# RishWijewardhena/vision-textile-inspection

Hardware: AMD Instinct MI355X
Metric: frames/sec whole-node, YOLOv8n-seg 640x640 bs=64; mask IoU vs CPU ref (higher is better)
Workload: dtype f16x2

## Files before the change

vision-textile-inspection_amd/csrc/conv_dev.h:

```cpp
#pragma once
#include "vti_internal.h"

namespace vti {

typedef _Float16 half_t;
typedef _Float16 half8 __attribute__((ext_vector_type(8)));
typedef _Float16 half4 __attribute__((ext_vector_type(4)));
typedef float f32x4 __attribute__((ext_vector_type(4)));

typedef unsigned u32x4 __attribute__((ext_vector_type(4)));

struct h2_t { unsigned u; };
struct h2x4 { u32x4 u; };
constexpr float H2_SX = 16.0f;

template <typename T> struct Tr;
template <> struct Tr<half_t> { typedef half8 vec; static constexpr int VEC = 8, KC = 32; static constexpr bool H16 = true, F32 = false, H2 = false; };
template <> struct Tr<float> { typedef f32x4 vec; static constexpr int VEC = 4, KC = 16; static constexpr bool H16 = false, F32 = true, H2 = false; };
template <> struct Tr<h2_t> { typedef h2x4 vec; static constexpr int VEC = 4, KC = 16; static constexpr bool H16 = false, F32 = false, H2 = true; };

typedef _Float16 half2v __attribute__((ext_vector_type(2)));
__device__ __forceinline__ unsigned h2_enc(float v) {
    half2v p;
    p[0] = (half_t)__builtin_fmaf(v, H2_SX, 0.0f);
// ... 20 lines not shown
    if constexpr (Tr<T>::H2) return (f32x4){h2_dec(u[0]), h2_dec(u[1]), h2_dec(u[2]), h2_dec(u[3])};
    else return __builtin_bit_cast(f32x4, u);
}
template <typename T> __device__ __forceinline__ f32x4 acc_bias(f32x4 acc, f32x4 bias, float alpha) {
    if constexpr (Tr<T>::H2) return acc * (f32x4){alpha, alpha, alpha, alpha} + bias;
    else return acc + bias;
}

__device__ __forceinline__ f32x4 mma(half8 w, half8 x, f32x4 c) {
    return __builtin_amdgcn_mfma_f32_16x16x32_f16(w, x, c, 0, 0, 0);
}
__device__ __forceinline__ f32x4 mma(f32x4 w, f32x4 x, f32x4 c) {
    c = __builtin_amdgcn_mfma_f32_16x16x4f32(w[0], x[0], c, 0, 0, 0);
    c = __builtin_amdgcn_mfma_f32_16x16x4f32(w[1], x[1], c, 0, 0, 0);
    c = __builtin_amdgcn_mfma_f32_16x16x4f32(w[2], x[2], c, 0, 0, 0);
    c = __builtin_amdgcn_mfma_f32_16x16x4f32(w[3], x[3], c, 0, 0, 0);
    return c;
}

__device__ __forceinline__ f32x4 mma(h2x4 w, h2x4 x, f32x4 c) {
    u32x4 wh, wl;
#pragma unroll
    for (int i = 0; i < 4; ++i) {
        wh[i] = __builtin_amdgcn_perm(w.u[i], w.u[i], 0x01000100u);
        wl[i] = w.u[i] >> 16;
    }
    const half8 xv = __builtin_bit_cast(half8, x.u);
    c = __builtin_amdgcn_mfma_f32_16x16x32_f16(__builtin_bit_cast(half8, wh), xv, c, 0, 0, 0);
    c = __builtin_amdgcn_mfma_f32_16x16x32_f16(__builtin_bit_cast(half8, wl), xv, c, 0, 0, 0);
    return c;
}

template <int NREP, int M, int TAPS, int XD, class LDX, class LDW>
__device__ __forceinline__ void h2_taps(f32x4 (&acc)[M][NREP], LDX ldx, LDW ldw) {
    constexpr int NSTEP = TAPS * M;
    constexpr unsigned SEL_H = 0x01000100u;
    h2x4 xq[XD];
    u32x4 wraw[NREP];
    u32x4 wh[2][NREP], wl[2][NREP];
#pragma unroll
    for (int n = 0; n < NREP; ++n) wraw[n] = ldw(0, n).u;
#pragma unroll
    for (int i = 0; i < XD - 1; ++i) xq[i] = ldx(i);
#pragma unroll
    for (int n = 0; n < NREP; ++n)
#pragma unroll
        for (int i = 0; i < 4; ++i) {
            wh[0][n][i] = __builtin_amdgcn_perm(wraw[n][i], wraw[n][i], SEL_H);
            wl[0][n][i] = wraw[n][i] >> 16;
        }
#pragma unroll
    for (int s_ = 0; s_ < NSTEP; ++s_) {
        const int tp = s_ / M, mm = s_ % M, cur = tp & 1, nxt = cur ^ 1;
#ifdef H2_EXP_NOXREAD
        if (s_ + XD - 1 < NSTEP && s_ < XD) xq[(s_ + XD - 1) % XD] = ldx(s_ + XD - 1);
#else
        if (s_ + XD - 1 < NSTEP) xq[(s_ + XD - 1) % XD] = ldx(s_ + XD - 1);
#endif
        if (mm == 0 && tp + 1 < TAPS) {
#pragma unroll
            for (int n = 0; n < NREP; ++n) wraw[n] = ldw(tp + 1, n).u;
        }
        __builtin_amdgcn_sched_barrier(0);
        const half8 xv = __builtin_bit_cast(half8, xq[s_ % XD].u);
#pragma unroll
        for (int j = 0; j < 2 * NREP; ++j) {
            const int n = j >> 1;
// ... 510 lines not shown
```

vision-textile-inspection_amd/csrc/conv_pk.hip:

```cpp
#include <algorithm>
#include <cstdlib>
#include <type_traits>

#include "conv_dev.h"

namespace vti {

constexpr int PK_PWP = 24;
constexpr int PK_TW = 20;
constexpr int PK_ROWS = 4;
constexpr int PK_MAXD = 9;
constexpr int PK_MAXD2 = 13;

using ConvPkS1 = Combos<Ints<1, 1>, Ints<2, 1>, Ints<3, 1>, Ints<4, 1>, Ints<5, 1>, Ints<1, 2>, Ints<2, 2>, Ints<3, 2>, Ints<4, 2>, Ints<1, 4>,
                        Ints<2, 4>>;
using ConvPkS2 = Combos<Ints<1, 4>, Ints<2, 2>, Ints<4, 1>, Ints<2, 1>, Ints<1, 2>>;
using Conv1Pk = decltype(concat(ConvPkS1{}, Combos<Ints<4, 4>>{}));
bool conv_pk_instantiated(int nrep, int wn) { return combo_has(ConvPkS1{}, nrep, wn); }
bool conv_pk2_instantiated(int nrep, int wn) { return combo_has(ConvPkS2{}, nrep, wn); }
bool conv1_pk_instantiated(int nrep, int wn) { return combo_has(Conv1Pk{}, nrep, wn); }
using Conv1PkWH2 = Combos<Ints<2, 2, 4>, Ints<2, 2, 6>, Ints<2, 2, 8>, Ints<2, 2, 12>, Ints<2, 2, 16>,
                          Ints<2, 4, 4>, Ints<2, 4, 6>, Ints<2, 4, 8>, Ints<2, 4, 12>, Ints<2, 4, 16>>;
using Conv1PkWF16 = Combos<Ints<2, 2, 2>, Ints<2, 2, 3>, Ints<2, 2, 4>, Ints<2, 2, 6>, Ints<2, 2, 8>,
                           Ints<2, 4, 2>, Ints<2, 4, 3>, Ints<2, 4, 4>, Ints<2, 4, 6>, Ints<2, 4, 8>, Ints<4, 1, 2>>;
// ... 20 lines not shown
static int pk_ring_depth(int maxd, int per_step, F lds_at) {
    int d = 2;
    while (d < maxd && lds_at(d + 1) <= 160 * 1024 && per_step * (d - 1) <= 63) ++d;
    return d;
}
static int pk3_depth(int S, int TH, int WN, int NREP, int nchunks, int wstat, int maxd) {
    if (!pk3_fits(S, TH, WN, NREP, nchunks, wstat)) return 0;
    const int ncomp = (TH / PK_ROWS) * WN;
    const int per_step = ((int)(pk_stage_bytes(TH, S) / 1024) + ncomp - 1) / ncomp + (nchunks > 2 && !wstat ? (WN * NREP * 9 + ncomp - 1) / ncomp : 0);
    return pk_ring_depth(maxd, per_step, [&](int d) { return pk3_lds_bytes(S, TH, WN, NREP, nchunks, d, wstat); });
}
size_t conv_pk_lds_bytes(int TH, int WN, int NREP, int nchunks, int depth, int wstat) { return pk3_lds_bytes(1, TH, WN, NREP, nchunks, depth, wstat); }
size_t conv_pk2_lds_bytes(int TH, int WN, int NREP, int nchunks, int depth, int wstat) { return pk3_lds_bytes(2, TH, WN, NREP, nchunks, depth, wstat); }
bool conv_pk_fits(int TH, int WN, int NREP, int nchunks, int wstat) { return pk3_fits(1, TH, WN, NREP, nchunks, wstat); }
bool conv_pk2_fits(int TH, int WN, int NREP, int nchunks, int wstat) { return pk3_fits(2, TH, WN, NREP, nchunks, wstat); }
int conv_pk_depth(int TH, int WN, int NREP, int nchunks, int wstat, int maxd) { return pk3_depth(1, TH, WN, NREP, nchunks, wstat, maxd); }
int conv_pk2_depth(int TH, int WN, int NREP, int nchunks, int wstat, int maxd) { return pk3_depth(2, TH, WN, NREP, nchunks, wstat, maxd); }

__device__ __forceinline__ void dma16(__amdgpu_buffer_rsrc_t r, unsigned voff, unsigned soff, unsigned lds_addr) {
    unsigned keep;
    asm volatile("s_mov_b32 %0, m0\n\ts_mov_b32 m0, %1\n\ts_nop 0\n\tbuffer_load_dwordx4 %2, %3, %4 offen lds\n\ts_mov_b32 m0, %0"
                 : "=&s"(keep) : "s"(lds_addr), "v"(voff), "s"(r), "s"(soff) : "memory");
}

template <int N> __device__ __forceinline__ void wait_vm() { asm volatile("s_waitcnt vmcnt(%0)" :: "i"(N) : "memory"); }
template <int N> struct WaitVm { static __device__ __forceinline__ void go(int n) { if (n >= N) wait_vm<N>(); else WaitVm<N - 1>::go(n); } };
template <> struct WaitVm<0> { static __device__ __forceinline__ void go(int) { wait_vm<0>(); } };

__device__ __forceinline__ void pk_stagger_wait(int units) {
    if (units > 0 && (int)(blockIdx.x >> 3) * 2 >= (int)(gridDim.x >> 3))
        for (int i = 0; i < units; ++i) __builtin_amdgcn_s_sleep(16);
}

template <typename T, int NREP, int WN, int NREP2 = 0, bool FOLD = false, int S = 1>
__global__ __launch_bounds__(512) void conv3_pk(const ConvParams p) {
    using vec = typename Tr<T>::vec;
    constexpr int VEC = Tr<T>::VEC, KC = Tr<T>::KC, ES = (int)sizeof(T);
    constexpr int TAPS = FOLD ? 4 : 9, NTB = WN * NREP;
    constexpr int PWP = S == 2 ? 2 * PK_PWP : PK_PWP;
    constexpr int MAXD = S == 2 ? PK_MAXD2 : PK_MAXD;
    static_assert(S == 1 || (S == 2 && !FOLD && NREP2 == 0), "stride 2: plain epilogue only");
    constexpr int WCHUNK = NTB * TAPS * 1024;
    constexpr unsigned OOB = 0x80000000u;
    constexpr bool FAST = !Tr<T>::F32;
    extern __shared__ __attribute__((aligned(16))) char smem[];

    const int tid = threadIdx.x, lane = tid & 63;
    const int wave = __builtin_amdgcn_readfirstlane(tid >> 6);
    static_assert(!FOLD || (WN == 4 && NREP2 > 0), "fold: one compute wave per output phase, fused 1x1 epilogue");
    const int ncomp = (p.TH / PK_ROWS) * WN;
    const int nld = (int)(blockDim.x >> 6) - ncomp;
    const int PH = S == 2 ? 2 * p.TH + 1 : p.TH + 2;
    const int stage_bytes = PH * PWP * 64;
    const int ndma = PH * PWP / 16;
    const int D = p.pk_depth;
    const bool stream_w = p.nchunks > 2 && !p.pk_wstat;
    const int wbuf_off = D * stage_bytes;
    const int bias_off = wbuf_off + (stream_w ? D : p.nchunks) * WCHUNK;
    const unsigned lds0 = (unsigned)(size_t)(__attribute__((address_space(3))) char*)smem;
    const int nt0 = blockIdx.y * NTB;

    for (int i = tid; i < NTB * 16; i += (int)blockDim.x) ((float*)(smem + bias_off))[i] = p.bias[nt0 * 16 + i];
    __syncthreads();

    int t, tend, tstride;
    if (p.pk_xcd) {
        const int per = (p.pk_tiles + 7) >> 3, k = blockIdx.x & 7;
        t = k * per + (int)(blockIdx.x >> 3);
        tend = min((k + 1) * per, p.pk_tiles);
        tstride = (int)(gridDim.x >> 3);
    } else {
        t = blockIdx.x; tend = p.pk_tiles; tstride = (int)gridDim.x;
    }
    if (t >= tend) return;
    auto tile_coords = [&](int tt, int& b, int& oy0, int& ox0) {
        const int tx = tt % p.tiles_x, r = tt / p.tiles_x;
        const int ty = r % p.tiles_y;
        b = r / p.tiles_y; oy0 = ty * p.TH; ox0 = tx * PK_TW;
    };
    const int nsteps = ((tend - t + tstride - 1) / tstride) * p.nchunks;

    if (wave >= ncomp) {
        const int lw = wave - ncomp;
        const int q = (lane & 3) ^ (((lane >> 4) & 1) << 1);
        const int cvalid = (p.Cin - q * VEC + KC - 1) / KC;
        int dyx[MAXD];
#pragma unroll
        for (int u = 0; u < MAXD; ++u) {
            const int s = (lw + u * nld) * 16 + (lane >> 2);
            if constexpr (S == 2) {
                const int py = (int)(((unsigned)s * 1366u) >> 16), r = s - py * PWP;
                const int plane = r >= PK_PWP ? 1 : 0, idx = r - plane * PK_PWP;
                dyx[u] = idx < PK_TW + 1 - plane ? (py << 8) | (2 * idx + plane) : -1;
            } else {
                const int py = (int)(((unsigned)s * 2731u) >> 16), px = s - py * PK_PWP;
                dyx[u] = px < PK_TW + 2 ? (py << 8) | px : -1;
            }
        }
        const __amdgpu_buffer_rsrc_t rsA = __builtin_amdgcn_make_buffer_rsrc((void*)p.in, 0, (int)p.in_bytes, 0x00020000);
        const __amdgpu_buffer_rsrc_t rsB = __builtin_amdgcn_make_buffer_rsrc((void*)p.wpk, 0, (int)p.wpk_bytes, 0x00020000);
        unsigned voff[MAXD];
        auto setup_voff = [&](int tt) {
            int b, oy0, ox0;
            tile_coords(tt, b, oy0, ox0);
#pragma unroll
            for (int u = 0; u < MAXD; ++u) {
                const int y = S * oy0 - 1 + (dyx[u] >> 8), x = S * ox0 - 1 + (dyx[u] & 255);
                const bool ok = dyx[u] >= 0 && (unsigned)y < (unsigned)p.Hin && (unsigned)x < (unsigned)p.Win;
                voff[u] = ok ? (unsigned)((((b * p.Hin + y) * p.Win + x) * p.in_ld + p.in_coff + q * VEC) * ES) : OOB;
            }
        };
        auto issue_patch = [&](int c, int stage) {
            const bool qok = c < cvalid;
            const unsigned dst = lds0 + stage * stage_bytes + lw * 1024;
#pragma unroll
            for (int u = 0; u < MAXD; ++u)
// ... 9 lines not shown
        int per_step = 0;
#pragma unroll
        for (int u = 0; u < MAXD; ++u) per_step += (lw + u * nld < ndma) ? 1 : 0;
        if (stream_w && lw < NTB * TAPS) per_step += (NTB * TAPS - lw + nld - 1) / nld;
        int it = t, ic = 0;
        setup_voff(t);
        auto issue_next = [&](int s) {
            const int stage = s % D;
            issue_patch(ic, stage);
            if (stream_w) issue_weights(ic, stage);
            if (++ic == p.nchunks) {
                ic = 0; it += tstride;
                if (it < tend) setup_voff(it);
            }
        };
        const int ahead = min(D - 1, nsteps);
        for (int s = 0; s < ahead; ++s) issue_next(s);
        int w1cnt = 0;
        if (!stream_w) {
            for (int c = 1; c < p.nchunks; ++c) {
                issue_weights(c, c);
                if (lw < NTB * TAPS) w1cnt += (NTB * TAPS - lw + nld - 1) / nld;
            }
        }
        for (int s = 0; s < nsteps; ++s) {
            const int inflight = min(D - 2, nsteps - 1 - s);
            WaitVm<63>::go(min(63, inflight * per_step + (s == 0 ? w1cnt : 0)));
            __builtin_amdgcn_s_barrier();
            if (s + D - 1 < nsteps) issue_next(s + D - 1);
        }
        return;
    }

    const int wn = wave % WN, wm = wave / WN;
    const int fpy = FOLD ? (wn >> 1) : 0, fpx = FOLD ? (wn & 1) : 0;
    int xa[MREP][3], ry[MREP], rx[MREP];
#pragma unroll
    for (int m = 0; m < MREP; ++m) {
        const int pp = m * 16 + (lane & 15), li = lane & 15;
        const int py = p.pk_lin ? (pp * 205) >> 12 : (m < 4 ? m : li >> 2);
        const int px = p.pk_lin ? pp - py * PK_TW : (m < 4 ? li : 16 + (li & 3));
        ry[m] = wm * PK_ROWS + py; rx[m] = px;
#pragma unroll
        for (int dx = 0; dx < 3; ++dx) {
            const int s = S == 2 ? (2 * ry[m]) * PWP + (dx == 1 ? PK_PWP + px : px + (dx >> 1))
                                 : (ry[m] + fpy) * PK_PWP + px + fpx + dx;
            xa[m][dx] = (s * 64 + (lane >> 4) * 16) ^ ((s & 4) << 3);
        }
    }
    const __amdgpu_buffer_rsrc_t rsO = __builtin_amdgcn_make_buffer_rsrc(p.out, 0, (int)p.out_bytes, 0x00020000);
    const __amdgpu_buffer_rsrc_t rsR = __builtin_amdgcn_make_buffer_rsrc((void*)p.res, 0, (int)p.res_bytes, 0x00020000);
    const bool fast_epi = NREP2 == 0 && !p.scalar_store && !p.out_f32 && !p.deconv_c &&
                          (sizeof(T) != 2 || NREP % 2 || (p.Cout & 7) == 0);
    int b, oy0, ox0;
    tile_coords(t, b, oy0, ox0);
    int step = 0;
    Stage2Regs<T, NREP, NREP2 ? NREP2 : 1> s2r;
    if constexpr (FOLD) stage2_preload<T, NREP, NREP2>(p, lane, true, s2r);
    VTI_STAMP(0);
    pk_stagger_wait(p.pk_stagger);
    while (true) {
        f32x4 acc[MREP][NREP];
#pragma unroll
        for (int m = 0; m < MREP; ++m)
#pragma unroll
            for (int n = 0; n < NREP; ++n) acc[m][n] = (f32x4){0.f, 0.f, 0.f, 0.f};
        for (int c = 0; c < p.nchunks; ++c, ++step) {
            const int cur = step % D;
            __builtin_amdgcn_s_barrier();
            asm volatile("" ::: "memory");
            if (step < 2) VTI_STAMP(1 + 4 * step);
            {
                const char* sx = smem + cur * stage_bytes;
                const char* sw = smem + wbuf_off + (stream_w ? cur : c) * WCHUNK + wn * (NREP * TAPS * 1024) + lane * 16;
                constexpr int NSTEP = TAPS * MREP;
                constexpr int XD = NREP >= 5 ? 3 : NREP == 4 ? 5 : NREP == 3 ? 5 : NREP == 2 ? 6 : 8, WD = 2;
                vec xq[XD];
                vec wq[WD][NREP];
                auto ldx = [&](int s_) -> vec {
                    const int tp = s_ / MREP, mm = s_ % MREP;
                    if constexpr (FOLD) return *(const vec*)(sx + xa[mm][tp & 1] + (tp >> 1) * (PK_PWP * 64));
                    else return *(const vec*)(sx + xa[mm][tp % 3] + (tp / 3) * (PWP * 64));
                };
                auto ldw = [&](int tp, vec (&w)[NREP]) {
#pragma unroll
                    for (int n = 0; n < NREP; ++n) w[n] = *(const vec*)(sw + (n * TAPS + tp) * 1024);
                };
                if constexpr (Tr<T>::H2) {
                    auto ldw1 = [&](int tp, int n) -> vec { return *(const vec*)(sw + (n * TAPS + tp) * 1024); };
#ifndef H2_XD
#define H2_XD (NREP >= 4 ? 3 : 4)
#endif
                    if constexpr (NREP >= 5) h2_taps_nmajor<NREP, MREP, TAPS>(acc, ldx, ldw1);
                    else h2_taps<NREP, MREP, TAPS, H2_XD>(acc, ldx, ldw1);
                } else {
                ldw(0, wq[0]);
#pragma unroll
                for (int i = 0; i < XD - 1; ++i) xq[i] = ldx(i);
#pragma unroll
                for (int s_ = 0; s_ < NSTEP; ++s_) {
                    const int tp = s_ / MREP, mm = s_ % MREP;
                    if (s_ + XD - 1 < NSTEP) xq[(s_ + XD - 1) % XD] = ldx(s_ + XD - 1);
                    if (mm == 0 && tp + 1 < TAPS) ldw(tp + 1, wq[(tp + 1) % WD]);
                    __builtin_amdgcn_sched_barrier(0);
#pragma unroll
                    for (int n = 0; n < NREP; ++n) acc[mm][n] = mma(wq[tp % WD][n], xq[s_ % XD], acc[mm][n]);
                    __builtin_amdgcn_sched_barrier(0);
                }
                }
            }
            if (step < 2) VTI_STAMP(3 + 4 * step);
        }
        VTI_STAMP(11);
        if (fast_epi) {
            const int crun = (nt0 + wn * NREP) * 16 + (lane >> 4) * 4 * NREP;
            const char* sb = smem + bias_off + (wn * NREP * 16 + (lane >> 4) * 4 * NREP) * 4;
            f32x4 bias_r[NREP];
#pragma unroll
            for (int n = 0; n < NREP; ++n) bias_r[n] = *(const f32x4*)(sb + n * 16);
            auto epi = [&](auto has_res_c) {
            constexpr bool has_res = decltype(has_res_c)::value;
            constexpr bool RES_UPFRONT = has_res && sizeof(T) == 2 && NREP <= 2;
            typedef unsigned u32x2 __attribute__((ext_vector_type(2)));
            u32x2 rr[RES_UPFRONT ? MREP : 1][RES_UPFRONT ? NREP : 1];
            if constexpr (RES_UPFRONT) {
#pragma unroll
                for (int m = 0; m < MREP; ++m) {
                    const int gy = oy0 + ry[m], gx = ox0 + rx[m];
                    const bool pv = gy < p.Hout && gx < p.Wout;
                    const int opix = (b * p.Hout + gy) * p.Wout + gx;
                    const unsigned rb = (unsigned)((opix * p.res_ld + p.res_coff + crun) * ES);
#pragma unroll
                    for (int n = 0; n < NREP; ++n)
                        rr[m][n] = __builtin_amdgcn_raw_buffer_load_b64(rsR, (pv && crun + 4 * n < p.Cout) ? rb + n * 8 : OOB, 0u, 0);
                }
            }
#pragma unroll
            for (int m = 0; m < MREP; ++m) {
                const int gy = oy0 + ry[m], gx = ox0 + rx[m];
                const bool pv = gy < p.Hout && gx < p.Wout;
                const int opix = (b * p.Hout + gy) * p.Wout + gx;
                const unsigned ob = (unsigned)((opix * p.out_ld + p.out_coff + crun) * ES);
                f32x4 v[NREP];
                if constexpr (RES_UPFRONT) {
#pragma unroll
                    for (int n = 0; n < NREP; ++n) {
                        const half4 r = __builtin_bit_cast(half4, rr[m][n]);
#pragma unroll
                        for (int j = 0; j < 4; ++j) v[n][j] = (float)r[j];
                    }
                } else if constexpr (has_res) {
                    const unsigned rb = (unsigned)((opix * p.res_ld + p.res_coff + crun) * ES);
#pragma unroll
                    for (int n = 0; n < NREP; ++n) {
                        const bool cv = pv && crun + 4 * n < p.Cout;
                        if constexpr (sizeof(T) == 2) {
                            const u32x2 r2 = __builtin_amdgcn_raw_buffer_load_b64(rsR, cv ? rb + n * 8 : OOB, 0u, 0);
                            const half4 r = __builtin_bit_cast(half4, r2);
#pragma unroll
                            for (int j = 0; j < 4; ++j) v[n][j] = (float)r[j];
                        } else {
                            v[n] = unpack4<T>(buf_load16<u32x4>(rsR, cv ? rb + n * 16 : OOB, 0u));
                        }
                    }
                }
#pragma unroll
                for (int n = 0; n < NREP; ++n) {
                    f32x4 a = acc_bias<T>(acc[m][n], bias_r[n], p.alpha);
                    if (p.act) a = silu4<FAST>(a);
                    if constexpr (has_res) v[n] += a; else v[n] = a;
                }
                if constexpr (sizeof(T) == 2 && NREP % 2 == 0) {
#pragma unroll
                    for (int n = 0; n < NREP; n += 2) {
                        half8 hv;
#pragma unroll
                        for (int j = 0; j < 4; ++j) { hv[j] = (half_t)v[n][j]; hv[4 + j] = (half_t)v[n + 1][j]; }
                        const bool cv = pv && crun + 4 * n + 8 <= p.Cout;
                        __builtin_amdgcn_raw_buffer_store_b128(__builtin_bit_cast(u32x4, hv), rsO, cv ? ob + n * 8 : OOB, 0u, 0);
                    }
                } else if constexpr (sizeof(T) == 2) {
                    typedef unsigned u32x2 __attribute__((ext_vector_type(2)));
#pragma unroll
                    for (int n = 0; n < NREP; ++n) {
                        half4 hv;
#pragma unroll
                        for (int j = 0; j < 4; ++j) hv[j] = (half_t)v[n][j];
                        const bool cv = pv && crun + 4 * n < p.Cout;
                        __builtin_amdgcn_raw_buffer_store_b64(__builtin_bit_cast(u32x2, hv), rsO, cv ? ob + n * 8 : OOB, 0u, 0);
                    }
                } else {
#pragma unroll
                    for (int n = 0; n < NREP; ++n) {
                        const bool cv = pv && crun + 4 * n < p.Cout;
                        __builtin_amdgcn_raw_buffer_store_b128(pack4<T>(v[n]), rsO, cv ? ob + n * 16 : OOB, 0u, 0);
                    }
                }
            }
            };
            if (p.has_res) epi(std::true_type{}); else epi(std::false_type{});
        } else {
            int opy[MREP], opx[MREP];
            bool pvalid[MREP];
#pragma unroll
            for (int m = 0; m < MREP; ++m) {
                opy[m] = oy0 + ry[m]; opx[m] = ox0 + rx[m];
                pvalid[m] = opy[m] < p.Hout && opx[m] < p.Wout;
            }
            if constexpr (FOLD) {
#pragma unroll
                for (int m = 0; m < MREP; ++m) { opy[m] = 2 * opy[m] + fpy; opx[m] = 2 * opx[m] + fpx; }
                const bool interior = oy0 > 0 && oy0 + p.TH < p.Hout && ox0 > 0 && ox0 + PK_TW < p.Wout;
                conv_stage2<T, NREP, NREP2, true, true>(p, acc, pvalid, opy, opx, b, lane, &s2r, interior);
            } else if constexpr (NREP2 == 0) conv_epilogue<T, NREP>(p, acc, pvalid, opy, opx, b, nt0, wn, lane);
            else conv_stage2<T, NREP, NREP2>(p, acc, pvalid, opy, opx, b, lane);
        }
        VTI_STAMP(12);
        const int tn = t + tstride;
        if (tn >= tend) break;
        t = tn;
        tile_coords(t, b, oy0, ox0);
    }
}


constexpr int PK1_MAXP = 5;

size_t conv1_pk_lds_bytes(int nwm, int WN, int NREP, int nchunks, int depth, int wstat, int cps) {
    const size_t stage = (size_t)nwm * 80 * 64 * cps;
    const size_t wch = (size_t)WN * NREP * 1024;
    const size_t wbytes = wstat == 2 ? 0 : wstat ? (size_t)nchunks * wch : (size_t)depth * wch * cps;
    return (size_t)depth * stage + wbytes + 1024  + (size_t)WN * NREP * 64;
}

template <typename V> __device__ __forceinline__ void reg_touch(V& v) {
    if constexpr (std::is_same<V, h2x4>::value) asm volatile("" : "+v"(v.u));
    else asm volatile("" : "+v"(v));
}

template <typename T, int NREP, int WN, int CPS, int NCH = 0>
__global__ __launch_bounds__(512) void conv1_pk(const ConvParams p) {
    using vec = typename Tr<T>::vec;
    constexpr int VEC = Tr<T>::VEC, KC = Tr<T>::KC, ES = (int)sizeof(T);
    constexpr int NTB = WN * NREP;
    constexpr int WCH = NTB * 1024;
    constexpr unsigned OOB = 0x80000000u;
    constexpr bool FAST = !Tr<T>::F32;
    extern __shared__ __attribute__((aligned(16))) char smem[];

    const int tid = threadIdx.x, lane = tid & 63;
    const int wave = __builtin_amdgcn_readfirstlane(tid >> 6);
    const int nwm = p.TH;
    const int ncomp = nwm * WN;
    const int nld = (int)(blockDim.x >> 6) - ncomp;
// ... 374 lines not shown
        }
        return combo_dispatch(Conv1Pk{}, [&](auto c) {
            using C = decltype(c);
            return launch_lds<conv1_pk<T, C::v[0], C::v[1], CPS>>(grid, dim3(threads), lds_bytes, st, p);
        }, nrep, p.WN);
    });
}

size_t conv_pk_fold_lds_bytes(int nchunks, int depth) { return depth * (size_t)6 * PK_PWP * 64 + (size_t)(nchunks > 1 ? 2 : 1) * 16 * 4 * 1024 + 16 * 16 * 4; }
int conv_pk_fold_depth(int nchunks, int maxd) {
    return pk_ring_depth(maxd, 0, [&](int d) { return conv_pk_fold_lds_bytes(nchunks, d); });
}

hipError_t launch_conv_pk_fold(int dtype, const ConvParams& p, size_t lds_bytes, hipStream_t st) {
    if (p.TH != 4 || p.TW != PK_TW || p.WN != 4 || p.nchunks > 2 || p.ntiles_n != 16 || !p.fold || !p.out2) return hipErrorInvalidValue;
    if (p.pk_wgs < 1 || (p.pk_xcd && p.pk_wgs % 8) || (size_t)p.in_bytes >= 0x80000000u) return hipErrorInvalidValue;
    if (p.pk_depth < 2 || p.pk_depth > 4 || lds_bytes < conv_pk_fold_lds_bytes(p.nchunks, p.pk_depth) || lds_bytes > 160 * 1024) return hipErrorInvalidValue;
    if (p.pk_tiles == 0) return hipSuccess;
    dim3 grid((unsigned)p.pk_wgs, 1);
    return combo_dispatch(FoldN2{}, [&](auto c) {
        return with_conv_type(dtype, [&](auto t) {
            return launch_lds<conv3_pk<typename decltype(t)::type, 4, 4, decltype(c)::v[0], true>>(grid, dim3(512), lds_bytes, st, p);
        });
    }, p.ntiles2);
}

hipError_t launch_conv_pk2(int dtype, int nrep, const ConvParams& p, size_t lds_bytes, hipStream_t st) {
    const int NTB = p.WN * nrep;
    if (p.TW != PK_TW || !conv_pk2_fits(p.TH, p.WN, nrep, p.nchunks, p.pk_wstat) || p.ntiles2 > 0) return hipErrorInvalidValue;
    if (p.pk_depth < 2 || p.pk_depth > 4 || lds_bytes < conv_pk2_lds_bytes(p.TH, p.WN, nrep, p.nchunks, p.pk_depth, p.pk_wstat) || lds_bytes > 160 * 1024) return hipErrorInvalidValue;
    if (p.ntiles_n % NTB || p.pk_wgs < 1 || (p.pk_xcd && p.pk_wgs % 8)) return hipErrorInvalidValue;
    if ((size_t)p.in_bytes >= 0x80000000u || (size_t)p.out_bytes >= 0x80000000u) return hipErrorInvalidValue;
    if (p.pk_tiles == 0) return hipSuccess;
    const int threads = 2 * (p.TH / PK_ROWS) * p.WN * 64;
    dim3 grid((unsigned)p.pk_wgs, (unsigned)(p.ntiles_n / NTB));
    return combo_dispatch(ConvPkS2{}, [&](auto c) {
        return with_conv_type(dtype, [&](auto t) {
            using C = decltype(c);
            return launch_lds<conv3_pk<typename decltype(t)::type, C::v[0], C::v[1], 0, false, 2>>(grid, dim3(threads), lds_bytes, st, p);
        });
    }, nrep, p.WN);
}

hipError_t launch_conv_pk(int dtype, int nrep, const ConvParams& p, size_t lds_bytes, hipStream_t st) {
    const int NTB = p.WN * nrep;
    if (p.TH % PK_ROWS || p.TW != PK_TW || !conv_pk_fits(p.TH, p.WN, nrep, p.nchunks, p.pk_wstat)) return hipErrorInvalidValue;
    if (p.pk_depth < 2 || p.pk_depth > 4 || lds_bytes < conv_pk_lds_bytes(p.TH, p.WN, nrep, p.nchunks, p.pk_depth, p.pk_wstat) || lds_bytes > 160 * 1024) return hipErrorInvalidValue;
    if (p.ntiles_n % NTB || p.pk_wgs < 1 || (p.pk_xcd && p.pk_wgs % 8)) return hipErrorInvalidValue;
    if ((size_t)p.in_bytes >= 0x80000000u || (size_t)p.out_bytes >= 0x80000000u) return hipErrorInvalidValue;
    if (p.pk_tiles == 0) return hipSuccess;
    const int threads = 2 * (p.TH / PK_ROWS) * p.WN * 64;
    dim3 grid((unsigned)p.pk_wgs, (unsigned)(p.ntiles_n / NTB));
    return with_conv_type(dtype, [&](auto t) {
        using T = typename decltype(t)::type;
        if (p.ntiles2 > 0) {
            if (p.WN != 1) return hipErrorInvalidValue;
            return combo_dispatch(FusedPairs{}, [&](auto c) {
                using C = decltype(c);
                return launch_lds<conv3_pk<T, C::v[0], 1, C::v[1]>>(grid, dim3(threads), lds_bytes, st, p);
            }, nrep, p.ntiles2);
        }
        return combo_dispatch(ConvPkS1{}, [&](auto c) {
            using C = decltype(c);
            return launch_lds<conv3_pk<T, C::v[0], C::v[1]>>(grid, dim3(threads), lds_bytes, st, p);
        }, nrep, p.WN);
    });
}

constexpr int BN_MREP1 = 7;

size_t bneck_pk_lds_bytes(int TH, int NREP, int depth) {
    return depth * (size_t)(TH + 4) * PK_PWP * 64 + (size_t)(TH + 2) * PK_PWP * 64 + 2 * (size_t)NREP * 9 * 1024 + 2 * (size_t)NREP * 64;
// ... 428 lines not shown
```

Measured before the change: 15580.

## Split stride-2 h2 conv M-tiles across paired compute waves with short-tap pipeline

For the h2 stride-2 conv3_pk variant with NREP=1 and WN=4, each output slot is now computed by two waves: one takes the first three M-repeats and the other takes the rest. The block grows to 768 threads to make room for the extra waves. A new h2_taps_short routine handles small M by interleaving the next tap's weight unpacking with the current tap's MFMAs, with double-buffered raw weight loads. The per-wave compute body moves into an include file so it can be instantiated over M sub-ranges. The aim is more latency hiding and shorter per-wave MFMA chains, at the cost of a larger block that may lower occupancy or increase register and LDS pressure.

```diff
diff --git a/vision-textile-inspection_amd/csrc/conv_dev.h b/vision-textile-inspection_amd/csrc/conv_dev.h
--- a/vision-textile-inspection_amd/csrc/conv_dev.h
+++ b/vision-textile-inspection_amd/csrc/conv_dev.h
@@ -76,7 +76,63 @@
 }
 
 template <int NREP, int M, int TAPS, int XD, class LDX, class LDW>
+__device__ __forceinline__ void h2_taps_short(f32x4 (&acc)[M][NREP], LDX ldx, LDW ldw) {
+    constexpr int NSTEP = TAPS * M;
+    constexpr unsigned SEL_H = 0x01000100u;
+    constexpr int PP = (4 + M - 1) / M;
+    static_assert(PP * 2 * M >= 8, "a tap's MFMAs cover the next tap's preparation");
+    h2x4 xq[XD];
+    u32x4 wraw[2][NREP];
+    u32x4 wh[2][NREP], wl[2][NREP];
+#pragma unroll
+    for (int n = 0; n < NREP; ++n) wraw[0][n] = ldw(0, n).u;
+#pragma unroll
+    for (int i = 0; i < XD - 1; ++i)
+        if (i < NSTEP) xq[i] = ldx(i);
+    if (TAPS > 1) {
+#pragma unroll
+        for (int n = 0; n < NREP; ++n) wraw[1][n] = ldw(1, n).u;
+    }
+#pragma unroll
+    for (int n = 0; n < NREP; ++n)
+#pragma unroll
+        for (int i = 0; i < 4; ++i) {
+            wh[0][n][i] = __builtin_amdgcn_perm(wraw[0][n][i], wraw[0][n][i], SEL_H);
+            wl[0][n][i] = wraw[0][n][i] >> 16;
+        }
+#pragma unroll
+    for (int s_ = 0; s_ < NSTEP; ++s_) {
+        const int tp = s_ / M, mm = s_ % M, cur = tp & 1, nxt = cur ^ 1;
+        if (s_ + XD - 1 < NSTEP) xq[(s_ + XD - 1) % XD] = ldx(s_ + XD - 1);
+        if (mm == 0 && tp + 2 < TAPS) {
+#pragma unroll
+            for (int n = 0; n < NREP; ++n) wraw[cur][n] = ldw(tp + 2, n).u;
+        }
+        __builtin_amdgcn_sched_barrier(0);
+        const half8 xv = __builtin_bit_cast(half8, xq[s_ % XD].u);
+#pragma unroll
+        for (int j = 0; j < 2 * NREP; ++j) {
+            const int n = j >> 1;
+            acc[mm][n] = __builtin_amdgcn_mfma_f32_16x16x32_f16(__builtin_bit_cast(half8, (j & 1) ? wl[cur][n] : wh[cur][n]), xv, acc[mm][n], 0, 0, 0);
+            const int k0 = (mm * 2 * NREP + j) * PP;
+            if (k0 < 8 * NREP && tp + 1 < TAPS) {
+#pragma unroll
+                for (int k = k0; k < k0 + PP; ++k) {
+                    const int pn = k >> 3, r = k & 7, i = r & 3;
+                    if (r < 4) wh[nxt][pn][i] = __builtin_amdgcn_perm(wraw[nxt][pn][i], wraw[nxt][pn][i], SEL_H);
+                    else wl[nxt][pn][i] = wraw[nxt][pn][i] >> 16;
+                }
+                __builtin_amdgcn_sched_group_barrier(0x008, 1, 0);
+                __builtin_amdgcn_sched_group_barrier(0x002, PP, 0);
+            }
+        }
+        __builtin_amdgcn_sched_barrier(0);
+    }
+}
+
+template <int NREP, int M, int TAPS, int XD, class LDX, class LDW>
 __device__ __forceinline__ void h2_taps(f32x4 (&acc)[M][NREP], LDX ldx, LDW ldw) {
+    if constexpr ((M - 1) * 2 < 8) { h2_taps_short<NREP, M, TAPS, XD>(acc, ldx, ldw); return; }
     constexpr int NSTEP = TAPS * M;
     constexpr unsigned SEL_H = 0x01000100u;
     h2x4 xq[XD];
diff --git a/vision-textile-inspection_amd/csrc/conv_pk.hip b/vision-textile-inspection_amd/csrc/conv_pk.hip
--- a/vision-textile-inspection_amd/csrc/conv_pk.hip
+++ b/vision-textile-inspection_amd/csrc/conv_pk.hip
@@ -76,8 +76,15 @@
         for (int i = 0; i < units; ++i) __builtin_amdgcn_s_sleep(16);
 }
 
+#ifndef VTI_PAIR_S2
+#define VTI_PAIR_S2 1
+#endif
+constexpr int PK_MA = 3;
+template <typename T, int NREP, int WN, int NREP2, bool FOLD, int S>
+constexpr bool PkPair = VTI_PAIR_S2 && Tr<T>::H2 && S == 2 && NREP == 1 && WN == 4 && NREP2 == 0 && !FOLD;
+
 template <typename T, int NREP, int WN, int NREP2 = 0, bool FOLD = false, int S = 1>
-__global__ __launch_bounds__(512) void conv3_pk(const ConvParams p) {
+__global__ __launch_bounds__((PkPair<T, NREP, WN, NREP2, FOLD, S> ? 768 : 512)) void conv3_pk(const ConvParams p) {
     using vec = typename Tr<T>::vec;
     constexpr int VEC = Tr<T>::VEC, KC = Tr<T>::KC, ES = (int)sizeof(T);
     constexpr int TAPS = FOLD ? 4 : 9, NTB = WN * NREP;
@@ -92,8 +99,10 @@
     const int tid = threadIdx.x, lane = tid & 63;
     const int wave = __builtin_amdgcn_readfirstlane(tid >> 6);
     static_assert(!FOLD || (WN == 4 && NREP2 > 0), "fold: one compute wave per output phase, fused 1x1 epilogue");
+    constexpr bool PAIR = PkPair<T, NREP, WN, NREP2, FOLD, S>;
     const int ncomp = (p.TH / PK_ROWS) * WN;
-    const int nld = (int)(blockDim.x >> 6) - ncomp;
+    const int ncw = PAIR ? 2 * ncomp : ncomp;
+    const int nld = (int)(blockDim.x >> 6) - ncw;
     const int PH = S == 2 ? 2 * p.TH + 1 : p.TH + 2;
     const int stage_bytes = PH * PWP * 64;
     const int ndma = PH * PWP / 16;
@@ -124,8 +133,8 @@
     };
     const int nsteps = ((tend - t + tstride - 1) / tstride) * p.nchunks;
 
-    if (wave >= ncomp) {
-        const int lw = wave - ncomp;
+    if (wave >= ncw) {
+        const int lw = wave - ncw;
         const int q = (lane & 3) ^ (((lane >> 4) & 1) << 1);
         const int cvalid = (p.Cin - q * VEC + KC - 1) / KC;
         int dyx[MAXD];
@@ -201,194 +210,17 @@
         return;
     }
 
-    const int wn = wave % WN, wm = wave / WN;
-    const int fpy = FOLD ? (wn >> 1) : 0, fpx = FOLD ? (wn & 1) : 0;
-    int xa[MREP][3], ry[MREP], rx[MREP];
-#pragma unroll
-    for (int m = 0; m < MREP; ++m) {
-        const int pp = m * 16 + (lane & 15), li = lane & 15;
-        const int py = p.pk_lin ? (pp * 205) >> 12 : (m < 4 ? m : li >> 2);
-        const int px = p.pk_lin ? pp - py * PK_TW : (m < 4 ? li : 16 + (li & 3));
-        ry[m] = wm * PK_ROWS + py; rx[m] = px;
-#pragma unroll
-        for (int dx = 0; dx < 3; ++dx) {
-            const int s = S == 2 ? (2 * ry[m]) * PWP + (dx == 1 ? PK_PWP + px : px + (dx >> 1))
-                                 : (ry[m] + fpy) * PK_PWP + px + fpx + dx;
-            xa[m][dx] = (s * 64 + (lane >> 4) * 16) ^ ((s & 4) << 3);
-        }
-    }
-    const __amdgpu_buffer_rsrc_t rsO = __builtin_amdgcn_make_buffer_rsrc(p.out, 0, (int)p.out_bytes, 0x00020000);
-    const __amdgpu_buffer_rsrc_t rsR = __builtin_amdgcn_make_buffer_rsrc((void*)p.res, 0, (int)p.res_bytes, 0x00020000);
-    const bool fast_epi = NREP2 == 0 && !p.scalar_store && !p.out_f32 && !p.deconv_c &&
-                          (sizeof(T) != 2 || NREP % 2 || (p.Cout & 7) == 0);
-    int b, oy0, ox0;
-    tile_coords(t, b, oy0, ox0);
-    int step = 0;
-    Stage2Regs<T, NREP, NREP2 ? NREP2 : 1> s2r;
-    if constexpr (FOLD) stage2_preload<T, NREP, NREP2>(p, lane, true, s2r);
-    VTI_STAMP(0);
-    pk_stagger_wait(p.pk_stagger);
-    while (true) {
-        f32x4 acc[MREP][NREP];
-#pragma unroll
-        for (int m = 0; m < MREP; ++m)
-#pragma unroll
-            for (int n = 0; n < NREP; ++n) acc[m][n] = (f32x4){0.f, 0.f, 0.f, 0.f};
-        for (int c = 0; c < p.nchunks; ++c, ++step) {
-            const int cur = step % D;
-            __builtin_amdgcn_s_barrier();
-            asm volatile("" ::: "memory");
-            if (step < 2) VTI_STAMP(1 + 4 * step);
-            {
-                const char* sx = smem + cur * stage_bytes;
-                const char* sw = smem + wbuf_off + (stream_w ? cur : c) * WCHUNK + wn * (NREP * TAPS * 1024) + lane * 16;
-                constexpr int NSTEP = TAPS * MREP;
-                constexpr int XD = NREP >= 5 ? 3 : NREP == 4 ? 5 : NREP == 3 ? 5 : NREP == 2 ? 6 : 8, WD = 2;
-                vec xq[XD];
-                vec wq[WD][NREP];
-                auto ldx = [&](int s_) -> vec {
-                    const int tp = s_ / MREP, mm = s_ % MREP;
-                    if constexpr (FOLD) return *(const vec*)(sx + xa[mm][tp & 1] + (tp >> 1) * (PK_PWP * 64));
-                    else return *(const vec*)(sx + xa[mm][tp % 3] + (tp / 3) * (PWP * 64));
-                };
-                auto ldw = [&](int tp, vec (&w)[NREP]) {
-#pragma unroll
-                    for (int n = 0; n < NREP; ++n) w[n] = *(const vec*)(sw + (n * TAPS + tp) * 1024);
-                };
-                if constexpr (Tr<T>::H2) {
-                    auto ldw1 = [&](int tp, int n) -> vec { return *(const vec*)(sw + (n * TAPS + tp) * 1024); };
-#ifndef H2_XD
-#define H2_XD (NREP >= 4 ? 3 : 4)
-#endif
-                    if constexpr (NREP >= 5) h2_taps_nmajor<NREP, MREP, TAPS>(acc, ldx, ldw1);
-                    else h2_taps<NREP, MREP, TAPS, H2_XD>(acc, ldx, ldw1);
-                } else {
-                ldw(0, wq[0]);
-#pragma unroll
-                for (int i = 0; i < XD - 1; ++i) xq[i] = ldx(i);
-#pragma unroll
-                for (int s_ = 0; s_ < NSTEP; ++s_) {
-                    const int tp = s_ / MREP, mm = s_ % MREP;
-                    if (s_ + XD - 1 < NSTEP) xq[(s_ + XD - 1) % XD] = ldx(s_ + XD - 1);
-                    if (mm == 0 && tp + 1 < TAPS) ldw(tp + 1, wq[(tp + 1) % WD]);
-                    __builtin_amdgcn_sched_barrier(0);
-#pragma unroll
-                    for (int n = 0; n < NREP; ++n) acc[mm][n] = mma(wq[tp % WD][n], xq[s_ % XD], acc[mm][n]);
-                    __builtin_amdgcn_sched_barrier(0);
-                }
-                }
-            }
-            if (step < 2) VTI_STAMP(3 + 4 * step);
-        }
-        VTI_STAMP(11);
-        if (fast_epi) {
-            const int crun = (nt0 + wn * NREP) * 16 + (lane >> 4) * 4 * NREP;
-            const char* sb = smem + bias_off + (wn * NREP * 16 + (lane >> 4) * 4 * NREP) * 4;
-            f32x4 bias_r[NREP];
-#pragma unroll
-            for (int n = 0; n < NREP; ++n) bias_r[n] = *(const f32x4*)(sb + n * 16);
-            auto epi = [&](auto has_res_c) {
-            constexpr bool has_res = decltype(has_res_c)::value;
-            constexpr bool RES_UPFRONT = has_res && sizeof(T) == 2 && NREP <= 2;
-            typedef unsigned u32x2 __attribute__((ext_vector_type(2)));
-            u32x2 rr[RES_UPFRONT ? MREP : 1][RES_UPFRONT ? NREP : 1];
-            if constexpr (RES_UPFRONT) {
-#pragma unroll
-                for (int m = 0; m < MREP; ++m) {
-                    const int gy = oy0 + ry[m], gx = ox0 + rx[m];
-                    const bool pv = gy < p.Hout && gx < p.Wout;
-                    const int opix = (b * p.Hout + gy) * p.Wout + gx;
-                    const unsigned rb = (unsigned)((opix * p.res_ld + p.res_coff + crun) * ES);
-#pragma unroll
-                    for (int n = 0; n < NREP; ++n)
-                        rr[m][n] = __builtin_amdgcn_raw_buffer_load_b64(rsR, (pv && crun + 4 * n < p.Cout) ? rb + n * 8 : OOB, 0u, 0);
-                }
-            }
-#pragma unroll
-            for (int m = 0; m < MREP; ++m) {
-                const int gy = oy0 + ry[m], gx = ox0 + rx[m];
-                const bool pv = gy < p.Hout && gx < p.Wout;
-                const int opix = (b * p.Hout + gy) * p.Wout + gx;
-                const unsigned ob = (unsigned)((opix * p.out_ld + p.out_coff + crun) * ES);
-                f32x4 v[NREP];
-                if constexpr (RES_UPFRONT) {
-#pragma unroll
-                    for (int n = 0; n < NREP; ++n) {
-                        const half4 r = __builtin_bit_cast(half4, rr[m][n]);
-#pragma unroll
-                        for (int j = 0; j < 4; ++j) v[n][j] = (float)r[j];
-                    }
-                } else if constexpr (has_res) {
-                    const unsigned rb = (unsigned)((opix * p.res_ld + p.res_coff + crun) * ES);
-#pragma unroll
-                    for (int n = 0; n < NREP; ++n) {
-                        const bool cv = pv && crun + 4 * n < p.Cout;
-                        if constexpr (sizeof(T) == 2) {
-                            const u32x2 r2 = __builtin_amdgcn_raw_buffer_load_b64(rsR, cv ? rb + n * 8 : OOB, 0u, 0);
-                            const half4 r = __builtin_bit_cast(half4, r2);
-#pragma unroll
-                            for (int j = 0; j < 4; ++j) v[n][j] = (float)r[j];
-                        } else {
-                            v[n] = unpack4<T>(buf_load16<u32x4>(rsR, cv ? rb + n * 16 : OOB, 0u));
-                        }
-                    }
-                }
-#pragma unroll
-                for (int n = 0; n < NREP; ++n) {
-                    f32x4 a = acc_bias<T>(acc[m][n], bias_r[n], p.alpha);
-                    if (p.act) a = silu4<FAST>(a);
-                    if constexpr (has_res) v[n] += a; else v[n] = a;
-                }
-                if constexpr (sizeof(T) == 2 && NREP % 2 == 0) {
-#pragma unroll
-                    for (int n = 0; n < NREP; n += 2) {
-                        half8 hv;
-#pragma unroll
-                        for (int j = 0; j < 4; ++j) { hv[j] = (half_t)v[n][j]; hv[4 + j] = (half_t)v[n + 1][j]; }
-                        const bool cv = pv && crun + 4 * n + 8 <= p.Cout;
-                        __builtin_amdgcn_raw_buffer_store_b128(__builtin_bit_cast(u32x4, hv), rsO, cv ? ob + n * 8 : OOB, 0u, 0);
-                    }
-                } else if constexpr (sizeof(T) == 2) {
-                    typedef unsigned u32x2 __attribute__((ext_vector_type(2)));
-#pragma unroll
-                    for (int n = 0; n < NREP; ++n) {
-                        half4 hv;
-#pragma unroll
-                        for (int j = 0; j < 4; ++j) hv[j] = (half_t)v[n][j];
-                        const bool cv = pv && crun + 4 * n < p.Cout;
-                        __builtin_amdgcn_raw_buffer_store_b64(__builtin_bit_cast(u32x2, hv), rsO, cv ? ob + n * 8 : OOB, 0u, 0);
-                    }
-                } else {
-#pragma unroll
-                    for (int n = 0; n < NREP; ++n) {
-                        const bool cv = pv && crun + 4 * n < p.Cout;
-                        __builtin_amdgcn_raw_buffer_store_b128(pack4<T>(v[n]), rsO, cv ? ob + n * 16 : OOB, 0u, 0);
-                    }
-                }
-            }
-            };
-            if (p.has_res) epi(std::true_type{}); else epi(std::false_type{});
+    if constexpr (PAIR) {
+        if (wave < ncomp) {
+            constexpr int M0 = 0, MN = PK_MA;
+#include "conv_pk3_compute.inc"
         } else {
-            int opy[MREP], opx[MREP];
-            bool pvalid[MREP];
-#pragma unroll
-            for (int m = 0; m < MREP; ++m) {
-                opy[m] = oy0 + ry[m]; opx[m] = ox0 + rx[m];
-                pvalid[m] = opy[m] < p.Hout && opx[m] < p.Wout;
-            }
-            if constexpr (FOLD) {
-#pragma unroll
-                for (int m = 0; m < MREP; ++m) { opy[m] = 2 * opy[m] + fpy; opx[m] = 2 * opx[m] + fpx; }
-                const bool interior = oy0 > 0 && oy0 + p.TH < p.Hout && ox0 > 0 && ox0 + PK_TW < p.Wout;
-                conv_stage2<T, NREP, NREP2, true, true>(p, acc, pvalid, opy, opx, b, lane, &s2r, interior);
-            } else if constexpr (NREP2 == 0) conv_epilogue<T, NREP>(p, acc, pvalid, opy, opx, b, nt0, wn, lane);
-            else conv_stage2<T, NREP, NREP2>(p, acc, pvalid, opy, opx, b, lane);
-        }
-        VTI_STAMP(12);
-        const int tn = t + tstride;
-        if (tn >= tend) break;
-        t = tn;
-        tile_coords(t, b, oy0, ox0);
+            constexpr int M0 = PK_MA, MN = MREP - PK_MA;
+#include "conv_pk3_compute.inc"
+        }
+    } else {
+        constexpr int M0 = 0, MN = MREP;
+#include "conv_pk3_compute.inc"
     }
 }
 
@@ -829,12 +661,14 @@
     if (p.ntiles_n % NTB || p.pk_wgs < 1 || (p.pk_xcd && p.pk_wgs % 8)) return hipErrorInvalidValue;
     if ((size_t)p.in_bytes >= 0x80000000u || (size_t)p.out_bytes >= 0x80000000u) return hipErrorInvalidValue;
     if (p.pk_tiles == 0) return hipSuccess;
-    const int threads = 2 * (p.TH / PK_ROWS) * p.WN * 64;
+    const int slots = (p.TH / PK_ROWS) * p.WN;
     dim3 grid((unsigned)p.pk_wgs, (unsigned)(p.ntiles_n / NTB));
     return combo_dispatch(ConvPkS2{}, [&](auto c) {
         return with_conv_type(dtype, [&](auto t) {
             using C = decltype(c);
-            return launch_lds<conv3_pk<typename decltype(t)::type, C::v[0], C::v[1], 0, false, 2>>(grid, dim3(threads), lds_bytes, st, p);
+            using T = typename decltype(t)::type;
+            const int threads = (PkPair<T, C::v[0], C::v[1], 0, false, 2> ? 3 : 2) * slots * 64;
+            return launch_lds<conv3_pk<T, C::v[0], C::v[1], 0, false, 2>>(grid, dim3(threads), lds_bytes, st, p);
         });
     }, nrep, p.WN);
 }
diff --git a/vision-textile-inspection_amd/csrc/conv_pk3_compute.inc b/vision-textile-inspection_amd/csrc/conv_pk3_compute.inc
--- /dev/null
+++ b/vision-textile-inspection_amd/csrc/conv_pk3_compute.inc
@@ -0,0 +1,208 @@
+    const int slot = PAIR ? wave % ncomp : wave;
+    const int wn = slot % WN, wm = slot / WN;
+    const int fpy = FOLD ? (wn >> 1) : 0, fpx = FOLD ? (wn & 1) : 0;
+    int xa[MN][3], ry[MN], rx[MN];
+#pragma unroll
+    for (int mi = 0; mi < MN; ++mi) {
+        const int m = M0 + mi;
+        const int pp = m * 16 + (lane & 15), li = lane & 15;
+        const int py = p.pk_lin ? (pp * 205) >> 12 : (m < 4 ? m : li >> 2);
+        const int px = p.pk_lin ? pp - py * PK_TW : (m < 4 ? li : 16 + (li & 3));
+        ry[mi] = wm * PK_ROWS + py; rx[mi] = px;
+#pragma unroll
+        for (int dx = 0; dx < 3; ++dx) {
+            const int s = S == 2 ? (2 * ry[mi]) * PWP + (dx == 1 ? PK_PWP + px : px + (dx >> 1))
+                                 : (ry[mi] + fpy) * PK_PWP + px + fpx + dx;
+            xa[mi][dx] = (s * 64 + (lane >> 4) * 16) ^ ((s & 4) << 3);
+        }
+    }
+    const __amdgpu_buffer_rsrc_t rsO = __builtin_amdgcn_make_buffer_rsrc(p.out, 0, (int)p.out_bytes, 0x00020000);
+    const __amdgpu_buffer_rsrc_t rsR = __builtin_amdgcn_make_buffer_rsrc((void*)p.res, 0, (int)p.res_bytes, 0x00020000);
+    const bool fast_epi = NREP2 == 0 && !p.scalar_store && !p.out_f32 && !p.deconv_c &&
+                          (sizeof(T) != 2 || NREP % 2 || (p.Cout & 7) == 0);
+    int b, oy0, ox0;
+    tile_coords(t, b, oy0, ox0);
+    int step = 0;
+    Stage2Regs<T, NREP, NREP2 ? NREP2 : 1> s2r;
+    if constexpr (FOLD) stage2_preload<T, NREP, NREP2>(p, lane, true, s2r);
+    VTI_STAMP(0);
+    pk_stagger_wait(p.pk_stagger);
+    while (true) {
+        f32x4 acc[MN][NREP];
+#pragma unroll
+        for (int m = 0; m < MN; ++m)
+#pragma unroll
+            for (int n = 0; n < NREP; ++n) acc[m][n] = (f32x4){0.f, 0.f, 0.f, 0.f};
+        for (int c = 0; c < p.nchunks; ++c, ++step) {
+            const int cur = step % D;
+            __builtin_amdgcn_s_barrier();
+            asm volatile("" ::: "memory");
+            if (step < 2) VTI_STAMP(1 + 4 * step);
+            {
+                const char* sx = smem + cur * stage_bytes;
+                const char* sw = smem + wbuf_off + (stream_w ? cur : c) * WCHUNK + wn * (NREP * TAPS * 1024) + lane * 16;
+                constexpr int NSTEP = TAPS * MN;
+                constexpr int XD = NREP >= 5 ? 3 : NREP == 4 ? 5 : NREP == 3 ? 5 : NREP == 2 ? 6 : 8, WD = 2;
+                vec xq[XD];
+                vec wq[WD][NREP];
+                auto ldx = [&](int s_) -> vec {
+                    const int tp = s_ / MN, mm = s_ % MN;
+                    if constexpr (FOLD) return *(const vec*)(sx + xa[mm][tp & 1] + (tp >> 1) * (PK_PWP * 64));
+                    else return *(const vec*)(sx + xa[mm][tp % 3] + (tp / 3) * (PWP * 64));
+                };
+                auto ldw = [&](int tp, vec (&w)[NREP]) {
+#pragma unroll
+                    for (int n = 0; n < NREP; ++n) w[n] = *(const vec*)(sw + (n * TAPS + tp) * 1024);
+                };
+                if constexpr (Tr<T>::H2) {
+                    auto ldw1 = [&](int tp, int n) -> vec { return *(const vec*)(sw + (n * TAPS + tp) * 1024); };
+#ifndef H2_XD
+#define H2_XD (NREP >= 4 ? 3 : 4)
+#endif
+#ifndef H2_XD_PAIR
+#define H2_XD_PAIR 4
+#endif
+                    if constexpr (NREP >= 5) h2_taps_nmajor<NREP, MN, TAPS>(acc, ldx, ldw1);
+                    else h2_taps<NREP, MN, TAPS, PAIR ? H2_XD_PAIR : H2_XD>(acc, ldx, ldw1);
+                } else {
+                ldw(0, wq[0]);
+#pragma unroll
+                for (int i = 0; i < XD - 1; ++i) xq[i] = ldx(i);
+#pragma unroll
+                for (int s_ = 0; s_ < NSTEP; ++s_) {
+                    const int tp = s_ / MN, mm = s_ % MN;
+                    if (s_ + XD - 1 < NSTEP) xq[(s_ + XD - 1) % XD] = ldx(s_ + XD - 1);
+                    if (mm == 0 && tp + 1 < TAPS) ldw(tp + 1, wq[(tp + 1) % WD]);
+                    __builtin_amdgcn_sched_barrier(0);
+#pragma unroll
+                    for (int n = 0; n < NREP; ++n) acc[mm][n] = mma(wq[tp % WD][n], xq[s_ % XD], acc[mm][n]);
+                    __builtin_amdgcn_sched_barrier(0);
+                }
+                }
+            }
+            if (step < 2) VTI_STAMP(3 + 4 * step);
+        }
+        VTI_STAMP(11);
+        if (fast_epi) {
+            const int crun = (nt0 + wn * NREP) * 16 + (lane >> 4) * 4 * NREP;
+            const char* sb = smem + bias_off + (wn * NREP * 16 + (lane >> 4) * 4 * NREP) * 4;
+            f32x4 bias_r[NREP];
+#pragma unroll
+            for (int n = 0; n < NREP; ++n) bias_r[n] = *(const f32x4*)(sb + n * 16);
+            auto epi = [&](auto has_res_c) {
+            constexpr bool has_res = decltype(has_res_c)::value;
+            constexpr bool RES_UPFRONT = has_res && sizeof(T) == 2 && NREP <= 2;
+            typedef unsigned u32x2 __attribute__((ext_vector_type(2)));
+            u32x2 rr[RES_UPFRONT ? MN : 1][RES_UPFRONT ? NREP : 1];
+            if constexpr (RES_UPFRONT) {
+#pragma unroll
+                for (int m = 0; m < MN; ++m) {
+                    const int gy = oy0 + ry[m], gx = ox0 + rx[m];
+                    const bool pv = gy < p.Hout && gx < p.Wout;
+                    const int opix = (b * p.Hout + gy) * p.Wout + gx;
+                    const unsigned rb = (unsigned)((opix * p.res_ld + p.res_coff + crun) * ES);
+#pragma unroll
+                    for (int n = 0; n < NREP; ++n)
+                        rr[m][n] = __builtin_amdgcn_raw_buffer_load_b64(rsR, (pv && crun + 4 * n < p.Cout) ? rb + n * 8 : OOB, 0u, 0);
+                }
+            }
+#pragma unroll
+            for (int m = 0; m < MN; ++m) {
+                const int gy = oy0 + ry[m], gx = ox0 + rx[m];
+                const bool pv = gy < p.Hout && gx < p.Wout;
+                const int opix = (b * p.Hout + gy) * p.Wout + gx;
+                const unsigned ob = (unsigned)((opix * p.out_ld + p.out_coff + crun) * ES);
+                f32x4 v[NREP];
+                if constexpr (RES_UPFRONT) {
+#pragma unroll
+                    for (int n = 0; n < NREP; ++n) {
+                        const half4 r = __builtin_bit_cast(half4, rr[m][n]);
+#pragma unroll
+                        for (int j = 0; j < 4; ++j) v[n][j] = (float)r[j];
+                    }
+                } else if constexpr (has_res) {
+                    const unsigned rb = (unsigned)((opix * p.res_ld + p.res_coff + crun) * ES);
+#pragma unroll
+                    for (int n = 0; n < NREP; ++n) {
+                        const bool cv = pv && crun + 4 * n < p.Cout;
+                        if constexpr (sizeof(T) == 2) {
+                            const u32x2 r2 = __builtin_amdgcn_raw_buffer_load_b64(rsR, cv ? rb + n * 8 : OOB, 0u, 0);
+                            const half4 r = __builtin_bit_cast(half4, r2);
+#pragma unroll
+                            for (int j = 0; j < 4; ++j) v[n][j] = (float)r[j];
+                        } else {
+                            v[n] = unpack4<T>(buf_load16<u32x4>(rsR, cv ? rb + n * 16 : OOB, 0u));
+                        }
+                    }
+                }
+#pragma unroll
+                for (int n = 0; n < NREP; ++n) {
+                    f32x4 a = acc_bias<T>(acc[m][n], bias_r[n], p.alpha);
+                    if (p.act) a = silu4<FAST>(a);
+                    if constexpr (has_res) v[n] += a; else v[n] = a;
+                }
+                if constexpr (sizeof(T) == 2 && NREP % 2 == 0) {
+#pragma unroll
+                    for (int n = 0; n < NREP; n += 2) {
+                        half8 hv;
+#pragma unroll
+                        for (int j = 0; j < 4; ++j) { hv[j] = (half_t)v[n][j]; hv[4 + j] = (half_t)v[n + 1][j]; }
+                        const bool cv = pv && crun + 4 * n + 8 <= p.Cout;
+                        __builtin_amdgcn_raw_buffer_store_b128(__builtin_bit_cast(u32x4, hv), rsO, cv ? ob + n * 8 : OOB, 0u, 0);
+                    }
+                } else if constexpr (sizeof(T) == 2) {
+                    typedef unsigned u32x2 __attribute__((ext_vector_type(2)));
+#pragma unroll
+                    for (int n = 0; n < NREP; ++n) {
+                        half4 hv;
+#pragma unroll
+                        for (int j = 0; j < 4; ++j) hv[j] = (half_t)v[n][j];
+                        const bool cv = pv && crun + 4 * n < p.Cout;
+                        __builtin_amdgcn_raw_buffer_store_b64(__builtin_bit_cast(u32x2, hv), rsO, cv ? ob + n * 8 : OOB, 0u, 0);
+                    }
+                } else {
+#pragma unroll
+                    for (int n = 0; n < NREP; ++n) {
+                        const bool cv = pv && crun + 4 * n < p.Cout;
+                        __builtin_amdgcn_raw_buffer_store_b128(pack4<T>(v[n]), rsO, cv ? ob + n * 16 : OOB, 0u, 0);
+                    }
+                }
+            }
+            };
+            if (p.has_res) epi(std::true_type{}); else epi(std::false_type{});
+        } else if constexpr (MN < MREP) {
+            f32x4 accf[MREP][NREP];
+            int opy[MREP], opx[MREP];
+            bool pvalid[MREP];
+#pragma unroll
+            for (int m = 0; m < MREP; ++m) {
+                const int mi = m - M0;
+                const bool mine = mi >= 0 && mi < MN;
+                opy[m] = mine ? oy0 + ry[mine ? mi : 0] : 0; opx[m] = mine ? ox0 + rx[mine ? mi : 0] : 0;
+                pvalid[m] = mine && opy[m] < p.Hout && opx[m] < p.Wout;
+#pragma unroll
+                for (int n = 0; n < NREP; ++n) accf[m][n] = mine ? acc[mine ? mi : 0][n] : (f32x4){0.f, 0.f, 0.f, 0.f};
+            }
+            conv_epilogue<T, NREP>(p, accf, pvalid, opy, opx, b, nt0, wn, lane);
+        } else {
+            int opy[MREP], opx[MREP];
+            bool pvalid[MREP];
+#pragma unroll
+            for (int m = 0; m < MREP; ++m) {
+                opy[m] = oy0 + ry[m]; opx[m] = ox0 + rx[m];
+                pvalid[m] = opy[m] < p.Hout && opx[m] < p.Wout;
+            }
+            if constexpr (FOLD) {
+#pragma unroll
+                for (int m = 0; m < MREP; ++m) { opy[m] = 2 * opy[m] + fpy; opx[m] = 2 * opx[m] + fpx; }
+                const bool interior = oy0 > 0 && oy0 + p.TH < p.Hout && ox0 > 0 && ox0 + PK_TW < p.Wout;
+                conv_stage2<T, NREP, NREP2, true, true>(p, acc, pvalid, opy, opx, b, lane, &s2r, interior);
+            } else if constexpr (NREP2 == 0) conv_epilogue<T, NREP>(p, acc, pvalid, opy, opx, b, nt0, wn, lane);
+            else conv_stage2<T, NREP, NREP2>(p, acc, pvalid, opy, opx, b, lane);
+        }
+        VTI_STAMP(12);
+        const int tn = t + tstride;
+        if (tn >= tend) break;
+        t = tn;
+        tile_coords(t, b, oy0, ox0);
+    }
```

Result: no change. 15430 (-0.9%).
